# momalekabid/clifford-vae

Hardware: NVIDIA B200
Metric: latent rsample+KL+bind samples/s (higher is better)
Workload: dtype f32

## Files before the change

clifford-vae_b200/clifford_b200/_lib.py:

```python
from __future__ import annotations

import ctypes as C
import os
import threading

import torch

_HERE = os.path.dirname(os.path.abspath(__file__))
LIB_PATH = os.environ.get("CLIFFORD_B200_LIB", os.path.join(_HERE, "libclifford_b200.so"))

_lib = None
_lock = threading.Lock()
_inited_devices: set[int] = set()

_f = C.c_void_p
_ll = C.c_longlong
_ull = C.c_ulonglong
_i = C.c_int
_fl = C.c_float
_db = C.c_double

_SIGNATURES = {
    "cvb_version": ([], _i),
    "cvb_last_error_string": ([], C.c_char_p),
    "cvb_init": ([], _i),
    "cvb_launch_count": ([], _ll),
    "cvb_clifford_ps_rsample": ([_f, _f, _ll, _i, _ll, _f, _f, _ull, _ull, _f, _f, _f, _f, _f, _ll, _i, _f], _i),
    "cvb_clifford_ps_rsample_bind": ([_f, _f, _ll, _f, _f, _ull, _ull, _f, _ll, _f, _f, _f, _f, _f, _ll, _i, _f], _i),
    "cvb_clifford_ps_rsample_log_prob": ([_f, _f, _ll, _f, _f, _ull, _ull, _f, _f, _f, _f, _ll, _i, _f], _i),
    "cvb_clifford_ps_rsample_backward": ([_f, _f, _f, _ll, _i, _ll, _f, _f, _f, _f, _f, _ll, _i, _f], _i),
    "cvb_clifford_ps_log_prob": ([_f, _f, _f, _ll, _i, _ll, _f, _f, _f, _f, _ll, _i, _f], _i),
    "cvb_clifford_spectrum_adjoint": ([_f, _f, _ll, _i, _f], _i),
    "cvb_ps_entropy_kl": ([_f, _ll, _i, _ll, _i, _db, _i, _db, _f, _f, _f, _f], _i),
    "cvb_clifford_vm_rsample": ([_f, _f, _ll, _i, _ll, _ull, _ull, _f, _ll, _i, _f], _i),
    "cvb_clifford_phases_to_vector": ([_f, _fl, _ull, _ull, _f, _ll, _i, _f], _i),
    "cvb_vsa_bind": ([_f, _f, _f, _ll, _ll, _ll, _i, _i, _f], _i),
    "cvb_vsa_depth_chain_cosine": ([_f, _f, _ll, _i, _i, _f], _i),
    "cvb_vsa_invert": ([_f, _f, _ll, _i, _f], _i),
    "cvb_vsa_permute": ([_f, _f, _f, _ll, _i, _i, _f], _i),
    "cvb_vsa_bundle_workspace_bytes": ([_ll, _i], _ll),
    "cvb_vsa_bundle": ([_f, _f, _ll, _i, _fl, _f, _f], _i),
    "cvb_vsa_cosine": ([_f, _f, _f, _ll, _ll, _ll, _i, _f], _i),
    "cvb_vsa_cosine_backward": ([_f, _f, _f, _f, _f, _ll, _ll, _ll, _i, _f], _i),
    "cvb_vsa_normalize": ([_f, _f, _ll, _i, _f], _i),
    "cvb_vsa_normalize_backward": ([_f, _f, _f, _ll, _i, _f], _i),
    "cvb_vsa_hrr_init": ([_f, _ll, _i, _ull, _ull, _f], _i),
    "cvb_vsa_unitary_init": ([_f, _ll, _i, _fl, _ull, _ull, _f], _i),
    "cvb_powerspherical_rsample": ([_f, _f, _ll, _f, _f, _ull, _ull, _f, _f, _ll, _i, _f], _i),
    "cvb_powerspherical_rsample_kl": ([_f, _f, _ll, _f, _f, _ull, _ull, _f, _f, _f, _f, _f, _ll, _i, _f], _i),
    "cvb_powerspherical_rsample_backward": ([_f, _f, _f, _ll, _f, _f, _f, _ull, _ull, _f, _f, _ll, _i, _f], _i),
    "cvb_powerspherical_log_prob": ([_f, _f, _f, _ll, _f, _f, _f, _ll, _i, _f], _i),
    "cvb_ps_log_normalizer": ([_f, _ll, _db, _f, _f, _f], _i),
    "cvb_sphere_uniform_rsample": ([_f, _ull, _ull, _f, _ll, _i, _fl, _f], _i),
    "cvb_vmf_rsample": ([_f, _f, _ll, _f, _f, _i, _f, _ull, _ull, _f, _f, _ll, _i, _f], _i),
    "cvb_vmf_rsample_kl": ([_f, _f, _ll, _f, _f, _i, _f, _ull, _ull, _f, _f, _f, _f, _f, _f, _f, _ll, _i, _f], _i),
    "cvb_vmf_rsample_backward": ([_f, _f, _f, _ll, _f, _f, _ull, _ull, _f, _f, _ll, _i, _f], _i),
    "cvb_vmf_entropy_lognorm": ([_f, _ll, _i, _f, _f, _f, _f, _f], _i),
    "cvb_clifford_ps_rsample_head": ([_f, _f, _ll, _fl, _fl, _f, _f, _ull, _ull, _f, _f, _f, _f, _f, _ll, _i, _f], _i),
    "cvb_clifford_ps_rsample_backward_head": ([_f, _f, _f, _ll, _fl, _fl, _f, _f, _f, _f, _f, _ll, _i, _f], _i),
    "cvb_powerspherical_rsample_kl_head": ([_f, _f, _ll, _fl, _fl, _f, _f, _ull, _ull, _f, _f, _f, _f, _f, _ll, _i, _f], _i),
    "cvb_powerspherical_rsample_backward_head": ([_f, _f, _f, _ll, _fl, _fl, _f, _f, _f, _ull, _ull, _f, _f, _ll, _i, _f], _i),
    "cvb_vmf_rsample_kl_head": ([_f, _f, _ll, _fl, _fl, _f, _f, _i, _f, _ull, _ull, _f, _f, _f, _f, _f, _f, _f, _ll, _i, _f], _i),
    "cvb_vmf_rsample_backward_head": ([_f, _f, _f, _ll, _fl, _fl, _f, _f, _ull, _ull, _f, _f, _ll, _i, _f], _i),
    "cvb_clifford_vm_entropy": ([_f, _ll, _i, _ll, _i, _f, _f, _f], _i),
    "cvb_vmf_log_prob": ([_f, _f, _f, _f, _ll, _f, _f, _ll, _i, _f], _i),
    "cvb_sphere_logprob_backward": ([_f, _f, _f, _ll, _f, _f, _ll, _i, _f], _i),
    "cvb_set_rng_device_counter": ([_f], _i),
    "cvb_set_rng_device_counter_autobump": ([_f], _i),
    "cvb_ps_halfangle_icdf_table": ([_f, _ll, _f, _f, _f], _i),
    "cvb_philox_fill": ([_f, _ll, _ull, _ull, _f], _i),
}

EXPORTED_SYMBOLS = tuple(_SIGNATURES)


class CliffordB200Error(RuntimeError):
    pass


def load():
    global _lib
    if _lib is not None:
        return _lib
    with _lock:
        if _lib is not None:
            return _lib
        if not os.path.exists(LIB_PATH):
            raise CliffordB200Error(
                f"{LIB_PATH} is missing: build it with `python -c 'import __graft_entry__ as g; g.build()'` "
                "(or `make -C clifford-vae_b200/csrc`). There is no CPU / PyTorch fallback for this path.")
        lib = C.CDLL(LIB_PATH)
        for name, (argtypes, restype) in _SIGNATURES.items():
            fn = getattr(lib, name)
            fn.argtypes = argtypes
            fn.restype = restype
        _lib = lib
    return _lib


def ensure_device(device: torch.device) -> None:
    if device.type != "cuda":
        raise CliffordB200Error(
            f"clifford_b200 ops run only on a CUDA (sm_100a) device, got a tensor on '{device}'. "
            "There is deliberately no CPU fallback; move the tensors to the GPU.")
    idx = device.index if device.index is not None else torch.cuda.current_device()
    if idx in _inited_devices:
        return
    lib = load()
    with torch.cuda.device(idx):
        rc = lib.cvb_init()
    if rc != 0:
        raise CliffordB200Error(f"cvb_init failed on cuda:{idx}: {lib.cvb_last_error_string().decode()}")
    _inited_devices.add(idx)


def check(rc: int, what: str) -> None:
    if rc != 0:
        msg = load().cvb_last_error_string().decode()
        if rc == 1:
            raise ValueError(f"{what}: {msg}")
        if rc == 2:
            raise NotImplementedError(f"{what}: {msg}")
# ... 110 lines not shown
```

clifford-vae_b200/csrc/api_core.cu:

```cuda
#include <cstdarg>
#include <cstring>
#include <mutex>
#include <unordered_map>
#include <vector>
#include "launch.cuh"
#include "icdf_table.cuh"
#include "../../include/clifford_b200.h"

namespace cvb {

static thread_local char g_err[512] = "";
std::atomic<long long> g_launch_count{0};
static std::mutex g_mu;
static const cplx* g_tw[64] = {nullptr};
static int g_sms[64] = {0};
static int* g_sched[64] = {nullptr};
static std::atomic<unsigned> g_sched_seq{0};
constexpr int kSchedSlots = 64;
static std::unordered_map<unsigned long long, size_t> g_smem_optin;
static std::unordered_map<unsigned long long, int> g_occ;
static unsigned long long func_key(const void* kernel) {
  int dev = 0;
  cudaGetDevice(&dev);
  return (unsigned long long)reinterpret_cast<uintptr_t>(kernel) * 64ull + (unsigned long long)(dev & 63);
// ... 122 lines not shown

unsigned int* rng_arrive_word() {
  int dev = 0;
  if (cudaGetDevice(&dev) != cudaSuccess || dev < 0 || dev >= 64 || !g_rng_autobump[dev]) return nullptr;
  return g_rng_arrive[dev];
}

int* next_sched_slot() {
  int dev = 0;
  if (cudaGetDevice(&dev) != cudaSuccess || dev < 0 || dev >= 64 || !g_sched[dev]) return nullptr;
  return g_sched[dev] + 2 * (g_sched_seq.fetch_add(1, std::memory_order_relaxed) % kSchedSlots);
}

int sm_count() {
  int dev = 0;
  cudaGetDevice(&dev);
  if (dev >= 0 && dev < 64 && g_sms[dev] > 0) return g_sms[dev];
  int n = 148;
  cudaDeviceGetAttribute(&n, cudaDevAttrMultiProcessorCount, dev);
  if (dev >= 0 && dev < 64) g_sms[dev] = n;
  return n;
}

int cached_ctas_per_sm(const void* kernel, int threads, size_t smem, bool* found) {
  std::lock_guard<std::mutex> lk(g_mu);
  auto it = g_occ.find(occ_key(kernel, threads, smem));
  *found = it != g_occ.end();
  return *found ? it->second : 0;
}
void store_ctas_per_sm(const void* kernel, int threads, size_t smem, int per_sm) {
  std::lock_guard<std::mutex> lk(g_mu);
  g_occ[occ_key(kernel, threads, smem)] = per_sm;
}
int ensure_smem_optin(const void* kernel, size_t smem) {
  if (smem <= 48 * 1024) return kOk;
  std::lock_guard<std::mutex> lk(g_mu);
  size_t& cur = g_smem_optin[func_key(kernel)];
  if (smem > cur) {
    CVB_CUDA(cudaFuncSetAttribute(kernel, cudaFuncAttributeMaxDynamicSharedMemorySize, (int)smem));
    cur = smem;
  }
  return kOk;
}

__global__ void philox_fill_kernel(uint4* out, long long n, PhiloxKey key) {
  for (long long i = (long long)blockIdx.x * blockDim.x + threadIdx.x; i < n; i += (long long)gridDim.x * blockDim.x)
    out[i] = philox4x32_10_rk(make_uint4((uint32_t)i, (uint32_t)(i >> 32), 0u, key.offset), key);
}

}

using namespace cvb;

extern "C" {

int cvb_version(void) { return 100; }
const char* cvb_last_error_string(void) { return g_err; }
long long cvb_launch_count(void) { return g_launch_count.load(); }

int cvb_init(void) {
  int dev = 0;
  CVB_CUDA(cudaGetDevice(&dev));
  CVB_REQUIRE(dev >= 0 && dev < 64, kUnsupported, "device ordinal %d out of range", dev);
  std::lock_guard<std::mutex> lk(g_mu);
  if (g_tw[dev]) return kOk;
  cudaDeviceProp prop;
  CVB_CUDA(cudaGetDeviceProperties(&prop, dev));
  CVB_REQUIRE(prop.major == 10, kUnsupported,
              "clifford_b200 is built for sm_100a only; device %d is sm_%d%d", dev, prop.major, prop.minor);
  std::vector<float2> host(kTwiddleEntries, make_float2(1.f, 0.f));
  for (int L = 4; L <= kTwiddleMaxLog2N; ++L) {
    const int N = 1 << L;
    for (int m = 0; m < N; ++m) {
      const double ang = -2.0 * 3.14159265358979323846264338327950288 * (double)m / (double)(2 * N);
      host[twiddle_offset(L) + m] = make_float2((float)cos(ang), (float)sin(ang));
    }
  }
  cplx* dptr = nullptr;
  CVB_CUDA(cudaMalloc(&dptr, sizeof(cplx) * kTwiddleEntries));
  CVB_CUDA(cudaMemcpy(dptr, host.data(), sizeof(cplx) * kTwiddleEntries, cudaMemcpyHostToDevice));
  int* sched = nullptr;
  CVB_CUDA(cudaMalloc(&sched, sizeof(int) * 2 * kSchedSlots));
  CVB_CUDA(cudaMemset(sched, 0, sizeof(int) * 2 * kSchedSlots));
  if (g_icdf_host.empty()) build_icdf_host(g_icdf_host);
  float2* icdf = nullptr;
  CVB_CUDA(cudaMalloc(&icdf, sizeof(float2) * kIcdfTableEntries));
  {
    std::vector<float2> dev_copy(g_icdf_host);
    for (auto& e : dev_copy) { e.x *= 2.0f; e.y *= 2.0f; }
    CVB_CUDA(cudaMemcpy(icdf, dev_copy.data(), sizeof(float2) * kIcdfTableEntries, cudaMemcpyHostToDevice));
  }
  g_icdf[dev] = icdf;
  g_sched[dev] = sched;
  unsigned int* arrive = nullptr;
  CVB_CUDA(cudaMalloc(&arrive, sizeof(unsigned int)));
  CVB_CUDA(cudaMemset(arrive, 0, sizeof(unsigned int)));
  g_rng_arrive[dev] = arrive;
  g_tw[dev] = dptr;
  g_sms[dev] = prop.multiProcessorCount;
  return kOk;
}

int cvb_set_rng_device_counter(const unsigned long long* counter) {
  int dev = 0;
  CVB_CUDA(cudaGetDevice(&dev));
  CVB_REQUIRE(dev >= 0 && dev < 64, kUnsupported, "device ordinal %d out of range", dev);
  g_rng_ctr[dev] = counter;
  g_rng_autobump[dev] = false;
  return kOk;
}

int cvb_set_rng_device_counter_autobump(unsigned long long* counter) {
  int dev = 0;
  CVB_CUDA(cudaGetDevice(&dev));
  CVB_REQUIRE(dev >= 0 && dev < 64, kUnsupported, "device ordinal %d out of range", dev);
  CVB_REQUIRE(counter == nullptr || g_rng_arrive[dev] != nullptr, kBadArgument, "cvb_set_rng_device_counter_autobump: call cvb_init() first");
  g_rng_ctr[dev] = counter;
  g_rng_autobump[dev] = counter != nullptr;
  return kOk;
}

int cvb_ps_halfangle_icdf_table(float* out, long long capacity_floats, int* n_kappa, int* n_nodes, float* kappa_max) {
  if (n_kappa) *n_kappa = kIcdfKappaNodes;
  if (n_nodes) *n_nodes = kIcdfCells + 1;
  if (kappa_max) *kappa_max = kIcdfKappaMax;
  if (!out) return kOk;
  const long long need = 2LL * kIcdfKappaNodes * (kIcdfCells + 1);
  CVB_REQUIRE(capacity_floats >= need, kBadArgument, "cvb_ps_halfangle_icdf_table: need room for %lld floats", need);
  {
    std::lock_guard<std::mutex> lk(g_mu);
    if (g_icdf_host.empty()) build_icdf_host(g_icdf_host);
  }
  for (int ki = 0; ki < kIcdfKappaNodes; ++ki)
    memcpy(out + 2LL * ki * (kIcdfCells + 1), g_icdf_host.data() + (size_t)ki * kIcdfRowStride, sizeof(float2) * (kIcdfCells + 1));
  return kOk;
}

int cvb_philox_fill(unsigned int* out, long long n_vec4, unsigned long long seed, unsigned long long offset,
                    void* stream) {
  CVB_REQUIRE(out && n_vec4 > 0, kBadArgument, "cvb_philox_fill: bad arguments");
  PhiloxKey key = make_key(seed, 0, 0);
  key.offset = (uint32_t)offset;
  key.dev_counter = nullptr;
  key.arrive = nullptr;
  philox_fill_kernel<<<148, 256, 0, (cudaStream_t)stream>>>(reinterpret_cast<uint4*>(out), n_vec4, key);
  return check_launch("philox_fill_kernel");
}

}
```

clifford-vae_b200/csrc/clifford_kernels.cuh:

```cuda
#pragma once
#include "fft_core.cuh"
#include "tma.cuh"
#include "rng.cuh"
#include "icdf_table.cuh"
#include "special.cuh"
#ifndef CVB_FWD_MINB
#define CVB_FWD_MINB 5
#endif
template <int LOG2N>
constexpr int clifford_bwd_min_blocks() { return LOG2N == 10 ? 4 : 5; }
#ifndef CVB_FWD_BIND_MINB
#define CVB_FWD_BIND_MINB 4
#endif
#ifndef CVB_FWD_KEEP_OWN
#define CVB_FWD_KEEP_OWN 1
#endif
#ifndef CVB_ICDF_LOOP_UNROLL
#define CVB_ICDF_LOOP_UNROLL 4
#endif
#ifndef CVB_FWD_LEAN_MINB
#define CVB_FWD_LEAN_MINB 6
#endif
template <int LOG2N, bool BIND = false, bool LEAN = false>
constexpr int clifford_fwd_min_blocks() {
// ... 465 lines not shown
          if (valid && k != 0) __sincosf(th, &x.y, &x.x);
          xch[pad16(k)] = x;
        }
      }
    } else {
#pragma unroll 4
      for (int e = 0; e < E; ++e) {
        const int k = t + e * T;
        cplx x = make_float2(1.0f, 0.0f);
        if (MODE == kSpectrum) {
          x = make_float2(0.f, 0.f);
          if (valid) {
            clifford_phasor<MODE, ROWK>(p, src, row, prow, k, gm, x);
            if (k == 0) x = make_float2(2.0f * x.x, 0.0f);
          }
        } else if (valid && k != 0) {
          clifford_phasor<MODE, ROWK>(p, src, row, prow, k, gm, x);
          if (MODE == kPsInjected && want_lp) lp_acc += circle_log_half_1pt<false>(src.tprime[k]);
        }
        xch[pad16(k)] = x;
      }
    }
    if (t == 0) xch[pad16(d)] = make_float2(MODE == kSpectrum ? 0.0f : 1.0f, 0.0f);
    if (MODE == kPsInjected && want_lp) lp_reduce();
    group_sync<LOG2N>();
    if (MODE == kPsInjected && want_lp) lp_emit();
    if (ICDF && table_row) {
      if (want_lp) { lp_reduce(); group_sync<LOG2N>(); lp_emit(); }
    } else if (MODE == kPsRng) {
      const int nq = *qcount;
#pragma unroll 1
      for (int i = t; i < nq; i += T) {
        const int k = queue[i];
        float tp_r;
        xch[pad16(k)] = clifford_phasor_retry<ROWK, LEAN>(p, src, row, prow, k, gm, tp_r);
        if (want_lp) lp_acc += circle_log_half_1pt<true>(tp_r);
      }
      if (want_lp) lp_reduce();
      group_sync<LOG2N>();
      if (want_lp) lp_emit();
      if (t == 0) *qcount = 0;
    }
    if (staged && t == 0 && next_row < p.rows) issue(next_row);
    if (ICDF && next_row < p.rows) {
      const float kn = fwd_row_kappa<LEAN || BIND>(p, next_row % p.loc_rows);
      if (icdf_row_ok(kn)) icdf_build_row<false, 1, true>(cells, kn + kEps, icdf, t, T);
    }
    cplx v[E];
    if (BIND) {
#pragma unroll
      for (int e = 0; e < E; ++e) spec[t + e * T] = xch[pad16(t + e * T)];
    }
    if (!BIND || p.z) {
      if constexpr (KEEP_OWN) {
        if (table_row) {
#pragma unroll
          for (int e = 0; e < E; ++e) v[e] = xown[KEEP_OWN ? e : 0];
          c2r_pretangle_load<LOG2N, true>(v, xch, t, tw);
        } else {
          c2r_pretangle_load<LOG2N>(v, xch, t, tw);
        }
      } else {
        c2r_pretangle_load<LOG2N>(v, xch, t, tw);
      }
      fft_run<LOG2N, true>(v, xch, t, tw);
      if (valid) {
        float2* zr = reinterpret_cast<float2*>(p.z + row * (2LL * d));
#pragma unroll
        for (int e = 0; e < E; ++e) stg_stream2(zr + t + e * T, v[e]);
      }
    }
    if (BIND) {
      const float2* br = reinterpret_cast<const float2*>(p.bind_b + (valid ? row % p.bind_b_rows : 0) * (2LL * d));
#pragma unroll
      for (int e = 0; e < E; ++e) v[e] = valid ? ldg_stream2(br + t + e * T) : make_float2(0.f, 0.f);
      fft_run<LOG2N, false>(v, xch, t, tw);
      group_sync<LOG2N>();
#pragma unroll
      for (int e = E / 2; e < E; ++e) xch[pad16(t + e * T)] = v[e];
      group_sync<LOG2N>();
      auto pair = [&](int k, int kp, cplx zb, cplx& vk, cplx& vkp) {
        constexpr float fold = 0.5f / (2.0f * d);
        const cplx zbp = cconj(kp == k ? zb : xch[pad16(kp)]);
        const cplx w = __ldg(&tw[twiddle_offset(LOG2N) + k]);
        const cplx sb = cadd(zb, zbp), db = cmul_mi(cmul(w, csub(zb, zbp)));
        const cplx Bk = cadd(sb, db), Bkp = cconj(csub(sb, db));
        const cplx Pk = cmul(spec[k], Bk), Pkpc = cconj(cmul(spec[kp], Bkp));
        const cplx s = cadd(Pk, Pkpc), q = cmul_i(cmul(cconj(w), csub(Pk, Pkpc)));
        vk = cadd_scaled(s, q, fold);
        vkp = cconj(cscale(csub(s, q), fold));
      };
#pragma unroll
      for (int e = 0; e < E / 2; ++e) {
        const int k = t + e * T, kp = (d - k) & (d - 1);
        cplx vkp;
        pair(k, kp, v[e], v[e], vkp);
        if (kp != k) spec[kp] = vkp;
      }
      if (t == 0) {
        cplx vk, vkp;
        pair(d / 2, d / 2, v[E / 2], vk, vkp);
        spec[d / 2] = vk;
      }
      group_sync<LOG2N>();
#pragma unroll
      for (int e = E / 2; e < E; ++e) v[e] = spec[t + e * T];
// ... 629 lines not shown
```

clifford-vae_b200/csrc/common.cuh:

```cuda
#pragma once
#include <cuda_runtime.h>
#include <cstdint>
#include <cmath>

#ifndef __CUDA_ARCH__
#define CVB_HOST_PASS 1
#endif

namespace cvb {

enum Status : int {
  kOk = 0,
  kBadArgument = 1,
  kUnsupported = 2,
  kCudaError = 3,
};

typedef float2 cplx;

__device__ __forceinline__ cplx cadd(cplx a, cplx b) { return __fadd2_rn(a, b); }
__device__ __forceinline__ cplx csub(cplx a, cplx b) { return __fadd2_rn(a, make_float2(-b.x, -b.y)); }
__device__ __forceinline__ cplx cmul(cplx a, cplx b) {
  return __ffma2_rn(b, make_float2(a.x, a.x), __fmul2_rn(make_float2(b.y, b.x), make_float2(-a.y, a.y)));
}
__device__ __forceinline__ cplx cmulc(cplx a, cplx b) {
  return __ffma2_rn(a, make_float2(b.x, b.x), __fmul2_rn(make_float2(a.y, a.x), make_float2(b.y, -b.y)));
}
__device__ __forceinline__ cplx cconj(cplx a) { return make_float2(a.x, -a.y); }
__device__ __forceinline__ cplx cscale(cplx a, float s) { return __fmul2_rn(a, make_float2(s, s)); }
__device__ __forceinline__ cplx cadd_scaled(cplx a, cplx b, float s) { return __fmul2_rn(__fadd2_rn(a, b), make_float2(s, s)); }
__device__ __forceinline__ cplx caxpy(float s, cplx a, cplx b) { return __ffma2_rn(a, make_float2(s, s), b); }
__device__ __forceinline__ cplx cmul_i(cplx a) { return make_float2(-a.y, a.x); }
__device__ __forceinline__ cplx cmul_mi(cplx a) { return make_float2(a.y, -a.x); }
__device__ __forceinline__ float cabs2(cplx a) { return fmaf(a.x, a.x, a.y * a.y); }

__host__ __device__ __forceinline__ constexpr int pad16(int i) { return i + (i >> 4); }

constexpr int kTwiddleMaxLog2N = 13;
constexpr int kTwiddleEntries = 1 << (kTwiddleMaxLog2N + 1);
__host__ __device__ __forceinline__ constexpr int twiddle_offset(int log2n) { return 1 << log2n; }

__device__ __forceinline__ float2 ldg_stream2(const float2* p) {
  float2 r;
  asm volatile("ld.global.nc.L1::no_allocate.v2.f32 {%0, %1}, [%2];" : "=f"(r.x), "=f"(r.y) : "l"(p));
  return r;
}
__device__ __forceinline__ float ldg_stream1(const float* p) {
  float r;
  asm volatile("ld.global.nc.L1::no_allocate.f32 %0, [%1];" : "=f"(r) : "l"(p));
  return r;
}
__device__ __forceinline__ void stg_stream2(float2* p, float2 v) {
  asm volatile("st.global.L1::no_allocate.v2.f32 [%0], {%1, %2};" ::"l"(p), "f"(v.x), "f"(v.y) : "memory");
}
__device__ __forceinline__ void stg_stream1(float* p, float v) {
  asm volatile("st.global.L1::no_allocate.f32 [%0], %1;" ::"l"(p), "f"(v) : "memory");
}

__device__ __forceinline__ void pdl_wait_and_release() {
  asm volatile("griddepcontrol.wait;" ::: "memory");
  asm volatile("griddepcontrol.launch_dependents;" ::: "memory");
}

__device__ __forceinline__ float fast_sqrt(float x) {
  float r;
  asm("sqrt.approx.ftz.f32 %0, %1;" : "=f"(r) : "f"(x));
  return r;
}

struct KappaHead {
  int on;
  float floor, kmax;
};
__device__ __forceinline__ float head_kappa(const KappaHead& h, float raw) {
  if (!h.on) return raw;
  const float sp = raw > 20.0f ? raw : log1pf(expf(raw));
  return fminf(sp + h.floor, h.kmax);
}
__device__ __forceinline__ float head_dkappa(const KappaHead& h, float raw) {
  if (!h.on) return 1.0f;
  const float e = expf(raw);
  const float sp = raw > 20.0f ? raw : log1pf(e);
  if (!(sp + h.floor <= h.kmax)) return 0.0f;
  return raw > 20.0f ? 1.0f : e / (e + 1.0f);
}

__device__ __forceinline__ float warp_sum(float v) {
#pragma unroll
  for (int o = 16; o > 0; o >>= 1) v += __shfl_xor_sync(0xffffffffu, v, o);
  return v;
}
__device__ __forceinline__ double warp_sum(double v) {
#pragma unroll
// ... 6 lines not shown
```

clifford-vae_b200/csrc/fft_core.cuh:

```cuda
#pragma once
#include "common.cuh"

namespace cvb {

constexpr int default_loge(int log2n) { return (log2n >= 8) ? 4 : (log2n >= 6 ? 3 : 2); }

template <int LOG2N_, int LOGE_, int MINTHREADS_ = 128>
struct FftPlanT {
  static_assert(LOG2N_ >= 4 && LOG2N_ <= 13, "fast path covers N = 16 .. 8192 complex points");
  static constexpr int LOG2N = LOG2N_;
  static constexpr int N = 1 << LOG2N;
  static constexpr int LOGE = LOGE_;
  static constexpr int E = 1 << LOGE;
  static constexpr int T = N / E;
  static constexpr int LOGT = LOG2N - LOGE;
  static constexpr int XCH = pad16(N) + 2;
  static constexpr int THREADS = (T >= MINTHREADS_) ? T : MINTHREADS_;
  static constexpr int GROUPS = THREADS / T;
};
template <int LOG2N>
using FftPlan = FftPlanT<LOG2N, default_loge(LOG2N)>;
template <int LOG2N>
using WideFftPlan = FftPlanT<LOG2N, (LOG2N >= 13) ? 5 : default_loge(LOG2N)>;

template <class Pl>
__device__ __forceinline__ void group_sync_p() {
  if constexpr (Pl::T <= 32) {
    __syncwarp();
  } else if constexpr (Pl::T < Pl::THREADS) {
    asm volatile("bar.sync %0, %1;" ::"r"(1 + (int)(threadIdx.x / Pl::T)), "n"(Pl::T) : "memory");
  } else {
    __syncthreads();
  }
}
template <int LOG2N>
__device__ __forceinline__ void group_sync() { group_sync_p<FftPlan<LOG2N>>(); }

template <bool INV>
__device__ __forceinline__ void dft2(cplx& a, cplx& b) {
  cplx t = a;
  a = cadd(t, b);
  b = csub(t, b);
}

template <bool INV>
__device__ __forceinline__ void dft4(cplx& a0, cplx& a1, cplx& a2, cplx& a3) {
  cplx s0 = cadd(a0, a2), d0 = csub(a0, a2);
  cplx s1 = cadd(a1, a3), d1 = csub(a1, a3);
  cplx r = INV ? cmul_i(d1) : cmul_mi(d1);
  a0 = cadd(s0, s1);
  a2 = csub(s0, s1);
  a1 = cadd(d0, r);
  a3 = csub(d0, r);
}

template <bool INV>
__device__ __forceinline__ cplx rot(cplx z, float c, float s) {
  return INV ? __ffma2_rn(z, make_float2(c, c), __fmul2_rn(make_float2(z.y, z.x), make_float2(-s, s)))
             : __ffma2_rn(z, make_float2(c, c), __fmul2_rn(make_float2(z.y, z.x), make_float2(s, -s)));
}

template <int R, bool INV>
struct Dft;

template <bool INV>
struct Dft<2, INV> {
  static __device__ __forceinline__ void run(cplx (&u)[2]) { dft2<INV>(u[0], u[1]); }
};
template <bool INV>
struct Dft<4, INV> {
  static __device__ __forceinline__ void run(cplx (&u)[4]) { dft4<INV>(u[0], u[1], u[2], u[3]); }
};
template <bool INV>
struct Dft<8, INV> {
  static __device__ __forceinline__ void run(cplx (&u)[8]) {
    constexpr float h = 0.70710678118654752440f;
    dft4<INV>(u[0], u[2], u[4], u[6]);
    dft4<INV>(u[1], u[3], u[5], u[7]);
    cplx o0 = u[1];
    cplx o1 = rot<INV>(u[3], h, h);
    cplx o2 = INV ? cmul_i(u[5]) : cmul_mi(u[5]);
    cplx o3 = rot<INV>(u[7], -h, h);
    cplx e0 = u[0], e1 = u[2], e2 = u[4], e3 = u[6];
    u[0] = cadd(e0, o0); u[4] = csub(e0, o0);
    u[1] = cadd(e1, o1); u[5] = csub(e1, o1);
    u[2] = cadd(e2, o2); u[6] = csub(e2, o2);
    u[3] = cadd(e3, o3); u[7] = csub(e3, o3);
  }
};
template <bool INV>
struct Dft<16, INV> {
  static __device__ __forceinline__ void run(cplx (&u)[16]) {
    constexpr float c1 = 0.92387953251128675613f, s1 = 0.38268343236508977173f;
    constexpr float h = 0.70710678118654752440f;
#pragma unroll
    for (int n1 = 0; n1 < 4; ++n1) dft4<INV>(u[n1], u[n1 + 4], u[n1 + 8], u[n1 + 12]);
    u[5] = rot<INV>(u[5], c1, s1);
    u[6] = rot<INV>(u[6], h, h);
    u[7] = rot<INV>(u[7], s1, c1);
    u[9] = rot<INV>(u[9], h, h);
    u[10] = INV ? cmul_i(u[10]) : cmul_mi(u[10]);
    u[11] = rot<INV>(u[11], -h, h);
    u[13] = rot<INV>(u[13], s1, c1);
    u[14] = rot<INV>(u[14], -h, h);
    u[15] = rot<INV>(u[15], -c1, -s1);
#pragma unroll
    for (int k2 = 0; k2 < 4; ++k2) dft4<INV>(u[4 * k2], u[4 * k2 + 1], u[4 * k2 + 2], u[4 * k2 + 3]);
    cplx t;
#define CVB_SWAP(a, b) t = u[a]; u[a] = u[b]; u[b] = t;
    CVB_SWAP(1, 4) CVB_SWAP(2, 8) CVB_SWAP(3, 12) CVB_SWAP(6, 9) CVB_SWAP(7, 13) CVB_SWAP(11, 14)
#undef CVB_SWAP
  }
};

template <bool INV>
struct Dft<32, INV> {
  static __device__ __forceinline__ void run(cplx (&u)[32]) {
    constexpr float c[16] = {1.0f, 0.98078528040323044913f, 0.92387953251128675613f, 0.83146961230254523708f,
                             0.70710678118654752440f, 0.55557023301960222474f, 0.38268343236508977173f, 0.19509032201612826785f,
                             0.0f, -0.19509032201612826785f, -0.38268343236508977173f, -0.55557023301960222474f,
                             -0.70710678118654752440f, -0.83146961230254523708f, -0.92387953251128675613f, -0.98078528040323044913f};
    constexpr float s[16] = {0.0f, 0.19509032201612826785f, 0.38268343236508977173f, 0.55557023301960222474f,
                             0.70710678118654752440f, 0.83146961230254523708f, 0.92387953251128675613f, 0.98078528040323044913f,
                             1.0f, 0.98078528040323044913f, 0.92387953251128675613f, 0.83146961230254523708f,
                             0.70710678118654752440f, 0.55557023301960222474f, 0.38268343236508977173f, 0.19509032201612826785f};
    cplx ev[16], od[16];
#pragma unroll
    for (int i = 0; i < 16; ++i) { ev[i] = u[2 * i]; od[i] = u[2 * i + 1]; }
    Dft<16, INV>::run(ev);
    Dft<16, INV>::run(od);
#pragma unroll
    for (int k = 0; k < 16; ++k) {
      cplx o;
      if (k == 0) o = od[0];
      else if (k == 8) o = INV ? cmul_i(od[8]) : cmul_mi(od[8]);
      else o = rot<INV>(od[k], c[k], s[k]);
      u[k] = cadd(ev[k], o);
      u[k + 16] = csub(ev[k], o);
    }
  }
};


template <bool INV>
struct Dft<64, INV> {
  static __device__ __forceinline__ void run(cplx (&u)[64]) {
    constexpr float C[17] = {1.0f, 0.99518472667219688624f, 0.98078528040323044913f, 0.95694033573220886494f,
                             0.92387953251128675613f, 0.88192126434835502971f, 0.83146961230254523708f, 0.77301045336273696081f,
                             0.70710678118654752440f, 0.63439328416364549822f, 0.55557023301960222474f, 0.47139673682599764856f,
                             0.38268343236508977173f, 0.29028467725446236764f, 0.19509032201612826785f, 0.09801714032956060199f, 0.0f};
#pragma unroll
    for (int n1 = 0; n1 < 8; ++n1) {
      cplx w[8];
#pragma unroll
      for (int j = 0; j < 8; ++j) w[j] = u[n1 + 8 * j];
      Dft<8, INV>::run(w);
#pragma unroll
      for (int j = 0; j < 8; ++j) u[n1 + 8 * j] = w[j];
    }
#pragma unroll
    for (int n1 = 1; n1 < 8; ++n1) {
#pragma unroll
      for (int k2 = 1; k2 < 8; ++k2) {
        const int m = n1 * k2;
        const int q = m >> 4, r = m & 15;
        const float c0 = C[r], s0 = C[16 - r];
        const float c = (q == 0) ? c0 : (q == 1) ? -s0 : (q == 2) ? -c0 : s0;
        const float sn = (q == 0) ? s0 : (q == 1) ? c0 : (q == 2) ? -s0 : -c0;
        cplx& z = u[n1 + 8 * k2];
        if (r == 0) {
          z = (q == 1) ? (INV ? cmul_i(z) : cmul_mi(z)) : (q == 2) ? make_float2(-z.x, -z.y) : (INV ? cmul_mi(z) : cmul_i(z));
        } else {
          z = rot<INV>(z, c, sn);
        }
      }
    }
#pragma unroll
    for (int k2 = 0; k2 < 8; ++k2) {
      cplx w[8];
#pragma unroll
      for (int j = 0; j < 8; ++j) w[j] = u[8 * k2 + j];
      Dft<8, INV>::run(w);
#pragma unroll
      for (int j = 0; j < 8; ++j) u[8 * k2 + j] = w[j];
    }
#pragma unroll
    for (int a = 0; a < 8; ++a) {
#pragma unroll
      for (int b = a + 1; b < 8; ++b) {
        const cplx tmp = u[a + 8 * b];
        u[a + 8 * b] = u[b + 8 * a];
        u[b + 8 * a] = tmp;
      }
    }
  }
};

template <int R>
__device__ __forceinline__ void apply_twiddle_powers(cplx (&u)[R], cplx w1) {
  if constexpr (R > 16) {
    cplx pw = w1, cur = w1;
#pragma unroll
    for (int i = 1; i < R; ++i) {
      if (i > 1) {
        if ((i & (i - 1)) == 0) { pw = cmul(pw, pw); cur = pw; }
        else cur = cmul(cur, w1);
      }
      u[i] = cmul(u[i], cur);
    }
    return;
  }
  cplx w[R];
  w[1] = w1;
#pragma unroll
  for (int i = 2; i < R; ++i) {
    if (i & 1) {
      w[i] = cmul(w[i - 1], w1);
    } else {
      w[i] = cmul(w[i >> 1], w[i >> 1]);
    }
  }
#pragma unroll
  for (int i = 1; i < R; ++i) u[i] = cmul(u[i], w[i]);
}

template <class Pl>
__device__ __forceinline__ void load_own_points(cplx (&v)[Pl::E], const cplx* xch, int t) {
  if constexpr (Pl::T % 16 == 0) {
    constexpr int S = Pl::T + Pl::T / 16;
    const cplx* xr = xch + pad16(t);
#pragma unroll
    for (int e = 0; e < Pl::E; ++e) v[e] = xr[e * S];
  } else {
#pragma unroll
    for (int e = 0; e < Pl::E; ++e) v[e] = xch[pad16(t + e * Pl::T)];
  }
}

template <class Pl, int P, bool INV, bool BASEPTR = false>
__device__ __forceinline__ void fft_pass_p(cplx (&v)[Pl::E], cplx* xch, const int t, const cplx* __restrict__ tw) {
  constexpr int LOG2N = Pl::LOG2N;
  constexpr int LOGNS = P * Pl::LOGE;
  constexpr int LOGR = (LOG2N - LOGNS) < Pl::LOGE ? (LOG2N - LOGNS) : Pl::LOGE;
  constexpr int R = 1 << LOGR, Q = Pl::E / R, NS = 1 << LOGNS;
  constexpr bool LAST = (LOGNS + LOGR == LOG2N);
  if (!LAST) group_sync_p<Pl>();
#pragma unroll
  for (int q = 0; q < Q; ++q) {
    cplx u[R];
#pragma unroll
    for (int r = 0; r < R; ++r) u[r] = v[q + r * Q];
    const int j = t + q * Pl::T;
    const int k = j & (NS - 1);
    if (P > 0) {
      cplx w1 = __ldg(&tw[twiddle_offset(LOG2N) + (k << (LOG2N + 1 - LOGNS - LOGR))]);
      if (INV) w1.y = -w1.y;
      apply_twiddle_powers<R>(u, w1);
    }
    Dft<R, INV>::run(u);
    if (LAST) {
#pragma unroll
      for (int r = 0; r < R; ++r) v[q + r * Q] = u[r];
    } else {
      const int j0 = ((j - k) << LOGR) + k;
#pragma unroll
      for (int r = 0; r < R; ++r) xch[pad16(j0 + r * NS)] = u[r];
    }
  }
  if constexpr (!LAST) {
    group_sync_p<Pl>();
    if constexpr (BASEPTR) {
      load_own_points<Pl>(v, xch, t);
    } else {
#pragma unroll
      for (int e = 0; e < Pl::E; ++e) v[e] = xch[pad16(t + e * Pl::T)];
    }
    fft_pass_p<Pl, P + 1, INV, BASEPTR>(v, xch, t, tw);
  }
}

template <class Pl, bool INV>
__device__ __forceinline__ void fft_run_p(cplx (&v)[Pl::E], cplx* xch, int t, const cplx* __restrict__ tw) {
  fft_pass_p<Pl, 0, INV>(v, xch, t, tw);
}
template <int LOG2N, bool INV>
__device__ __forceinline__ void fft_run(cplx (&v)[FftPlan<LOG2N>::E], cplx* xch, int t,
                                        const cplx* __restrict__ tw) {
  fft_pass_p<FftPlan<LOG2N>, 0, INV, true>(v, xch, t, tw);
}

template <int LOG2N>
__device__ __forceinline__ float r2c_untangle(cplx (&v)[FftPlan<LOG2N>::E], cplx* xch, int t,
                                              const cplx* __restrict__ tw) {
  using Pl = FftPlan<LOG2N>;
  constexpr int N = Pl::N;
  if constexpr (Pl::T % 16 == 0) {
    constexpr int S = Pl::T + Pl::T / 16;
    cplx* xk = xch + pad16(t);
    const cplx* xm = xch + pad16(N - t);
    const cplx* twp = tw + twiddle_offset(LOG2N) + t;
    group_sync<LOG2N>();
#pragma unroll
    for (int e = 0; e < Pl::E; ++e) xk[e * S] = v[e];
    group_sync<LOG2N>();
    const float nyq0 = v[0].x - v[0].y;
#pragma unroll
    for (int e = 0; e < Pl::E; ++e) {
      const cplx z = v[e];
      const cplx* pp = (e == 0) ? ((t == 0) ? xch : xm) : xm - e * S;
      const cplx zp = cconj(*pp);
      const cplx w = __ldg(twp + e * Pl::T);
      const cplx s = cadd(z, zp), d = csub(z, zp);
      const cplx wd = cmul_mi(cmul(w, d));
      v[e] = cadd_scaled(s, wd, 0.5f);
    }
    return nyq0;
  }
  group_sync<LOG2N>();
#pragma unroll
  for (int e = 0; e < Pl::E; ++e) xch[pad16(t + e * Pl::T)] = v[e];
  group_sync<LOG2N>();
  const float nyq = v[0].x - v[0].y;
#pragma unroll
  for (int e = 0; e < Pl::E; ++e) {
    const int k = t + e * Pl::T;
    const cplx z = v[e];
    const cplx zp = cconj(xch[pad16((N - k) & (N - 1))]);
    const cplx w = __ldg(&tw[twiddle_offset(LOG2N) + k]);
    const cplx s = cadd(z, zp), d = csub(z, zp);
    const cplx wd = cmul_mi(cmul(w, d));
    v[e] = cadd_scaled(s, wd, 0.5f);
  }
  return nyq;
}

template <int LOG2N>
__device__ __forceinline__ void c2r_pretangle(cplx (&v)[FftPlan<LOG2N>::E], float x_nyq, cplx* xch, int t,
                                              const cplx* __restrict__ tw) {
  using Pl = FftPlan<LOG2N>;
  constexpr int N = Pl::N;
  constexpr float scale = 1.0f / (2.0f * N);
  group_sync<LOG2N>();
#pragma unroll
  for (int e = 0; e < Pl::E; ++e) xch[pad16(t + e * Pl::T)] = v[e];
  if (t == 0) xch[pad16(N)] = make_float2(x_nyq, 0.0f);
  group_sync<LOG2N>();
#pragma unroll
  for (int e = 0; e < Pl::E; ++e) {
    const int k = t + e * Pl::T;
    const cplx x = v[e];
    const cplx xp = cconj(xch[pad16(N - k)]);
    const cplx w = cconj(__ldg(&tw[twiddle_offset(LOG2N) + k]));
    const cplx s = cadd(x, xp), d = csub(x, xp);
    const cplx wd = cmul_i(cmul(w, d));
    v[e] = cadd_scaled(s, wd, scale);
  }
}

template <int LOG2N, bool OWN = false>
__device__ __forceinline__ void c2r_pretangle_load(cplx (&v)[FftPlan<LOG2N>::E], const cplx* xch, int t,
                                                   const cplx* __restrict__ tw) {
  using Pl = FftPlan<LOG2N>;
  constexpr int N = Pl::N;
  constexpr float scale = 1.0f / (2.0f * N);
  if constexpr (Pl::T % 16 == 0) {
    constexpr int S = Pl::T + Pl::T / 16;
    const cplx* xk = xch + pad16(t);
    const cplx* xm = xch + pad16(N - t);
    const cplx* twp = tw + twiddle_offset(LOG2N) + t;
#pragma unroll
    for (int e = 0; e < Pl::E; ++e) {
      const cplx x = OWN ? v[e] : xk[e * S];
      const cplx xp = cconj(xm[-e * S]);
      const cplx w = cconj(__ldg(twp + e * Pl::T));
      const cplx s = cadd(x, xp), d = csub(x, xp);
      const cplx wd = cmul_i(cmul(w, d));
      v[e] = cadd_scaled(s, wd, scale);
    }
    return;
  }
#pragma unroll
  for (int e = 0; e < Pl::E; ++e) {
    const int k = t + e * Pl::T;
    const cplx x = OWN ? v[e] : xch[pad16(k)];
    const cplx xp = cconj(xch[pad16(N - k)]);
    const cplx w = cconj(__ldg(&tw[twiddle_offset(LOG2N) + k]));
    const cplx s = cadd(x, xp), d = csub(x, xp);
    const cplx wd = cmul_i(cmul(w, d));
    v[e] = cadd_scaled(s, wd, scale);
  }
}

template <int LOG2N>
__device__ __forceinline__ float group_sum(float val, float* scratch, int t) {
  constexpr int T = FftPlan<LOG2N>::T;
  constexpr int W = T < 32 ? T : 32;
#pragma unroll
  for (int o = W / 2; o > 0; o >>= 1) val += __shfl_xor_sync(0xffffffffu, val, o);
  if constexpr (T > 32) {
    group_sync<LOG2N>();
    if ((t & 31) == 0) scratch[t >> 5] = val;
    group_sync<LOG2N>();
    float s = 0.f;
#pragma unroll
    for (int i = 0; i < T / 32; ++i) s += scratch[i];
    val = s;
  }
  return val;
}

}
```

include/clifford_b200.h:

```cpp
#ifndef CLIFFORD_B200_H_
#define CLIFFORD_B200_H_

#if defined(__GNUC__)
#define CVB_API __attribute__((visibility("default")))
#else
#define CVB_API
#endif

#ifdef __cplusplus
extern "C" {
#endif

enum cvb_status { CVB_OK = 0, CVB_BAD_ARGUMENT = 1, CVB_UNSUPPORTED = 2, CVB_CUDA_ERROR = 3 };

enum cvb_bind_mode {
  CVB_BIND_MUL = 0,
  CVB_BIND_MUL_CONJ = 1,
  CVB_BIND_DIV = 2,
  CVB_BIND_DIV_CONJ = 3,
  CVB_BIND_NEG_MUL_CONJ = 4
};

CVB_API int cvb_version(void);
CVB_API const char* cvb_last_error_string(void);
// ... 81 lines not shown
                            unsigned long long offset, float* z, float* save, long long rows, int D, void* stream);
CVB_API int cvb_vmf_rsample_kl(const float* loc, const float* kappa, long long loc_rows, const double* e_rounds,
                               const double* u_rounds, int n_rounds, const float* gnoise, unsigned long long seed,
                               unsigned long long offset, float* z, float* save, float* entropy, float* kl,
                               float* dentropy, float* log_norm, float* dlog_norm, long long rows, int D, void* stream);
CVB_API int cvb_vmf_rsample_backward(const float* grad_z, const float* loc, const float* kappa, long long loc_rows,
                                     const float* gnoise, const float* save, unsigned long long seed,
                                     unsigned long long offset, float* dloc, float* dkappa, long long rows, int D,
                                     void* stream);
CVB_API int cvb_vmf_entropy_lognorm(const float* kappa, long long rows, int D, float* entropy, float* log_norm,
                                    float* dentropy, float* dlog_norm, void* stream);

CVB_API int cvb_clifford_vm_entropy(const float* kappa, long long kappa_row_stride, int kappa_el_stride, long long rows,
                                    int d, float* entropy, float* dentropy, void* stream);
CVB_API int cvb_vmf_log_prob(const float* value, const float* loc, const float* kappa, const float* log_norm,
                             long long loc_rows, float* log_prob, float* dot, long long rows, int D, void* stream);
CVB_API int cvb_sphere_logprob_backward(const float* w, const float* value, const float* loc, long long loc_rows,
                                        float* dvalue, float* dloc, long long rows, int D, void* stream);

CVB_API int cvb_clifford_ps_rsample_head(const float* loc, const float* raw_scale, long long loc_rows, float floor, float kmax,
                                         const float* tprime, const float* gnoise, unsigned long long seed,
                                         unsigned long long offset, float* z, float* tp_signed, float* entropy, float* kl,
                                         float* dentropy_draw, long long rows, int d, void* stream);
CVB_API int cvb_clifford_ps_rsample_backward_head(const float* grad_z, const float* loc, const float* raw_scale,
                                                  long long loc_rows, float floor, float kmax, const float* tprime,
                                                  const float* gnoise, const float* tp_signed, float* dloc,
                                                  float* draw_scale, long long rows, int d, void* stream);
CVB_API int cvb_powerspherical_rsample_kl_head(const float* loc, const float* raw_scale, long long loc_rows, float floor,
                                               float kmax, const float* tprime, const float* gnoise,
                                               unsigned long long seed, unsigned long long offset, float* z, float* save,
                                               float* entropy, float* kl, float* dentropy_draw, long long rows, int D,
                                               void* stream);
CVB_API int cvb_powerspherical_rsample_backward_head(const float* grad_z, const float* loc, const float* raw_scale,
                                                     long long loc_rows, float floor, float kmax, const float* tprime,
                                                     const float* gnoise, const float* save, unsigned long long seed,
                                                     unsigned long long offset, float* dloc, float* draw_scale,
                                                     long long rows, int D, void* stream);
CVB_API int cvb_vmf_rsample_kl_head(const float* loc, const float* raw_scale, long long loc_rows, float floor, float kmax,
                                    const double* e_rounds, const double* u_rounds, int n_rounds, const float* gnoise,
                                    unsigned long long seed, unsigned long long offset, float* z, float* save,
                                    float* entropy, float* kl, float* dentropy_draw, float* log_norm,
                                    float* dlog_norm_draw, long long rows, int D, void* stream);
CVB_API int cvb_vmf_rsample_backward_head(const float* grad_z, const float* loc, const float* raw_scale, long long loc_rows,
                                          float floor, float kmax, const float* gnoise, const float* save,
                                          unsigned long long seed, unsigned long long offset, float* dloc,
                                          float* draw_scale, long long rows, int D, void* stream);

CVB_API int cvb_set_rng_device_counter(const unsigned long long* counter);
CVB_API int cvb_set_rng_device_counter_autobump(unsigned long long* counter);

CVB_API int cvb_ps_halfangle_icdf_table(float* out, long long capacity_floats, int* n_kappa, int* n_nodes,
                                        float* kappa_max);

CVB_API int cvb_philox_fill(unsigned int* out, long long n_vec4, unsigned long long seed, unsigned long long offset,
                    void* stream);

#ifdef __cplusplus
}
#endif
#endif
```

Baseline: 34.16 million.

## Precompute FFT stage twiddle powers in table and restructure radix-8/16 butterflies with FMAs

```diff
diff --git a/clifford-vae_b200/clifford_b200/_lib.py b/clifford-vae_b200/clifford_b200/_lib.py
--- a/clifford-vae_b200/clifford_b200/_lib.py
+++ b/clifford-vae_b200/clifford_b200/_lib.py
@@ -68,6 +68,7 @@
     "cvb_set_rng_device_counter": ([_f], _i),
     "cvb_set_rng_device_counter_autobump": ([_f], _i),
     "cvb_ps_halfangle_icdf_table": ([_f, _ll, _f, _f, _f], _i),
+    "cvb_fft_twiddle_table": ([_f, _ll, _f], _i),
     "cvb_philox_fill": ([_f, _ll, _ull, _ull, _f], _i),
 }
 
diff --git a/clifford-vae_b200/csrc/api_core.cu b/clifford-vae_b200/csrc/api_core.cu
--- a/clifford-vae_b200/csrc/api_core.cu
+++ b/clifford-vae_b200/csrc/api_core.cu
@@ -198,6 +198,32 @@
 
 using namespace cvb;
 
+static float2 unit_root(long long m, long long M) {
+  const long long q = (4 * m) / M, r = m - q * (M / 4);
+  const double a = 2.0 * 3.14159265358979323846264338327950288 * (double)r / (double)M;
+  const double c = cos(a), s = -sin(a);
+  const double x = (q == 0) ? c : (q == 1) ? s : (q == 2) ? -c : -s;
+  const double y = (q == 0) ? s : (q == 1) ? -c : (q == 2) ? -s : c;
+  return make_float2((float)x, (float)y);
+}
+
+static void build_twiddle_host(std::vector<float2>& host) {
+  host.assign(kTwiddleTableEntries, make_float2(1.f, 0.f));
+  for (int L = 4; L <= kTwiddleMaxLog2N; ++L) {
+    const int N = 1 << L;
+    for (int m = 0; m < N; ++m) {
+      const double ang = -2.0 * 3.14159265358979323846264338327950288 * (double)m / (double)(2 * N);
+      host[twiddle_offset(L) + m] = make_float2((float)cos(ang), (float)sin(ang));
+    }
+  }
+  for (int logr = 1; logr <= kPowerMaxLog2R; ++logr)
+    for (int logns = 1; logns + logr <= kTwiddleMaxLog2N; ++logns) {
+      const int NS = 1 << logns, R = 1 << logr;
+      for (int j = 0; j < logr; ++j)
+        for (int k = 0; k < NS; ++k) host[power_offset(logns, logr) + j * NS + k] = unit_root((long long)k << j, (long long)NS * R);
+    }
+}
+
 extern "C" {
 
 int cvb_version(void) { return 100; }
@@ -214,17 +240,11 @@
   CVB_CUDA(cudaGetDeviceProperties(&prop, dev));
   CVB_REQUIRE(prop.major == 10, kUnsupported,
               "clifford_b200 is built for sm_100a only; device %d is sm_%d%d", dev, prop.major, prop.minor);
-  std::vector<float2> host(kTwiddleEntries, make_float2(1.f, 0.f));
-  for (int L = 4; L <= kTwiddleMaxLog2N; ++L) {
-    const int N = 1 << L;
-    for (int m = 0; m < N; ++m) {
-      const double ang = -2.0 * 3.14159265358979323846264338327950288 * (double)m / (double)(2 * N);
-      host[twiddle_offset(L) + m] = make_float2((float)cos(ang), (float)sin(ang));
-    }
-  }
+  std::vector<float2> host;
+  build_twiddle_host(host);
   cplx* dptr = nullptr;
-  CVB_CUDA(cudaMalloc(&dptr, sizeof(cplx) * kTwiddleEntries));
-  CVB_CUDA(cudaMemcpy(dptr, host.data(), sizeof(cplx) * kTwiddleEntries, cudaMemcpyHostToDevice));
+  CVB_CUDA(cudaMalloc(&dptr, sizeof(cplx) * kTwiddleTableEntries));
+  CVB_CUDA(cudaMemcpy(dptr, host.data(), sizeof(cplx) * kTwiddleTableEntries, cudaMemcpyHostToDevice));
   int* sched = nullptr;
   CVB_CUDA(cudaMalloc(&sched, sizeof(int) * 2 * kSchedSlots));
   CVB_CUDA(cudaMemset(sched, 0, sizeof(int) * 2 * kSchedSlots));
@@ -282,6 +302,17 @@
   return kOk;
 }
 
+int cvb_fft_twiddle_table(float* out, long long capacity_floats, long long* n_entries) {
+  if (n_entries) *n_entries = kTwiddleTableEntries;
+  if (!out) return kOk;
+  CVB_REQUIRE(capacity_floats >= 2LL * kTwiddleTableEntries, kBadArgument,
+              "cvb_fft_twiddle_table: need room for %lld floats", 2LL * kTwiddleTableEntries);
+  std::vector<float2> host;
+  build_twiddle_host(host);
+  memcpy(out, host.data(), sizeof(float2) * kTwiddleTableEntries);
+  return kOk;
+}
+
 int cvb_philox_fill(unsigned int* out, long long n_vec4, unsigned long long seed, unsigned long long offset,
                     void* stream) {
   CVB_REQUIRE(out && n_vec4 > 0, kBadArgument, "cvb_philox_fill: bad arguments");
diff --git a/clifford-vae_b200/csrc/clifford_kernels.cuh b/clifford-vae_b200/csrc/clifford_kernels.cuh
--- a/clifford-vae_b200/csrc/clifford_kernels.cuh
+++ b/clifford-vae_b200/csrc/clifford_kernels.cuh
@@ -541,6 +541,9 @@
       for (int e = 0; e < E; ++e) spec[t + e * T] = xch[pad16(t + e * T)];
     }
     if (!BIND || p.z) {
+#ifdef CVB_PAIR_PRETANGLE
+      if (BIND) group_sync<LOG2N>();
+#endif
       if constexpr (KEEP_OWN) {
         if (table_row) {
 #pragma unroll
diff --git a/clifford-vae_b200/csrc/common.cuh b/clifford-vae_b200/csrc/common.cuh
--- a/clifford-vae_b200/csrc/common.cuh
+++ b/clifford-vae_b200/csrc/common.cuh
@@ -39,6 +39,14 @@
 constexpr int kTwiddleMaxLog2N = 13;
 constexpr int kTwiddleEntries = 1 << (kTwiddleMaxLog2N + 1);
 __host__ __device__ __forceinline__ constexpr int twiddle_offset(int log2n) { return 1 << log2n; }
+
+constexpr int kPowerMaxLog2R = 4;
+__host__ __device__ __forceinline__ constexpr int power_offset(int logns, int logr) {
+  int off = kTwiddleEntries;
+  for (int b = 1; b < logr; ++b) off += b * ((1 << (kTwiddleMaxLog2N + 1 - b)) - 2);
+  return off + logr * ((1 << logns) - 2);
+}
+constexpr int kTwiddleTableEntries = power_offset(kTwiddleMaxLog2N + 1 - kPowerMaxLog2R, kPowerMaxLog2R);
 
 __device__ __forceinline__ float2 ldg_stream2(const float2* p) {
   float2 r;
diff --git a/clifford-vae_b200/csrc/fft_core.cuh b/clifford-vae_b200/csrc/fft_core.cuh
--- a/clifford-vae_b200/csrc/fft_core.cuh
+++ b/clifford-vae_b200/csrc/fft_core.cuh
@@ -72,40 +72,67 @@
   static __device__ __forceinline__ void run(cplx (&u)[4]) { dft4<INV>(u[0], u[1], u[2], u[3]); }
 };
 template <bool INV>
+__device__ __forceinline__ cplx jrot(cplx z) { return INV ? cmul_i(z) : cmul_mi(z); }
+__device__ __forceinline__ void fma_pm(cplx a, cplx z, float s, cplx& plus, cplx& minus) {
+  plus = __ffma2_rn(z, make_float2(s, s), a);
+  minus = __ffma2_rn(z, make_float2(-s, -s), a);
+}
+
+template <bool INV>
 struct Dft<8, INV> {
   static __device__ __forceinline__ void run(cplx (&u)[8]) {
     constexpr float h = 0.70710678118654752440f;
     dft4<INV>(u[0], u[2], u[4], u[6]);
     dft4<INV>(u[1], u[3], u[5], u[7]);
-    cplx o0 = u[1];
-    cplx o1 = rot<INV>(u[3], h, h);
-    cplx o2 = INV ? cmul_i(u[5]) : cmul_mi(u[5]);
-    cplx o3 = rot<INV>(u[7], -h, h);
-    cplx e0 = u[0], e1 = u[2], e2 = u[4], e3 = u[6];
+    const cplx o1 = cadd(u[3], jrot<INV>(u[3]));
+    const cplx o2 = jrot<INV>(u[5]);
+    const cplx o3 = csub(jrot<INV>(u[7]), u[7]);
+    const cplx o0 = u[1];
+    const cplx e0 = u[0], e1 = u[2], e2 = u[4], e3 = u[6];
     u[0] = cadd(e0, o0); u[4] = csub(e0, o0);
-    u[1] = cadd(e1, o1); u[5] = csub(e1, o1);
+    fma_pm(e1, o1, h, u[1], u[5]);
     u[2] = cadd(e2, o2); u[6] = csub(e2, o2);
-    u[3] = cadd(e3, o3); u[7] = csub(e3, o3);
+    fma_pm(e3, o3, h, u[3], u[7]);
   }
 };
 template <bool INV>
 struct Dft<16, INV> {
   static __device__ __forceinline__ void run(cplx (&u)[16]) {
-    constexpr float c1 = 0.92387953251128675613f, s1 = 0.38268343236508977173f;
+    constexpr float c1 = 0.92387953251128675613f;
+    constexpr float tn = 0.41421356237309504880f;
     constexpr float h = 0.70710678118654752440f;
 #pragma unroll
     for (int n1 = 0; n1 < 4; ++n1) dft4<INV>(u[n1], u[n1 + 4], u[n1 + 8], u[n1 + 12]);
-    u[5] = rot<INV>(u[5], c1, s1);
-    u[6] = rot<INV>(u[6], h, h);
-    u[7] = rot<INV>(u[7], s1, c1);
-    u[9] = rot<INV>(u[9], h, h);
-    u[10] = INV ? cmul_i(u[10]) : cmul_mi(u[10]);
-    u[11] = rot<INV>(u[11], -h, h);
-    u[13] = rot<INV>(u[13], s1, c1);
-    u[14] = rot<INV>(u[14], -h, h);
-    u[15] = rot<INV>(u[15], -c1, -s1);
-#pragma unroll
-    for (int k2 = 0; k2 < 4; ++k2) dft4<INV>(u[4 * k2], u[4 * k2 + 1], u[4 * k2 + 2], u[4 * k2 + 3]);
+    dft4<INV>(u[0], u[1], u[2], u[3]);
+    {
+      const cplx a2 = cadd(u[6], jrot<INV>(u[6]));
+      cplx s0, d0;
+      fma_pm(u[4], a2, h, s0, d0);
+      const cplx b1 = __ffma2_rn(jrot<INV>(u[5]), make_float2(tn, tn), u[5]);
+      const cplx b3 = __ffma2_rn(u[7], make_float2(tn, tn), jrot<INV>(u[7]));
+      const cplx s1 = cadd(b1, b3), d1 = csub(b1, b3);
+      fma_pm(s0, s1, c1, u[4], u[6]);
+      fma_pm(d0, jrot<INV>(d1), c1, u[5], u[7]);
+    }
+    {
+      const cplx a2 = jrot<INV>(u[10]);
+      const cplx s0 = cadd(u[8], a2), d0 = csub(u[8], a2);
+      const cplx b1 = cadd(u[9], jrot<INV>(u[9]));
+      const cplx b3 = csub(jrot<INV>(u[11]), u[11]);
+      const cplx s1 = cadd(b1, b3), d1 = csub(b1, b3);
+      fma_pm(s0, s1, h, u[8], u[10]);
+      fma_pm(d0, jrot<INV>(d1), h, u[9], u[11]);
+    }
+    {
+      const cplx a2 = csub(jrot<INV>(u[14]), u[14]);
+      cplx s0, d0;
+      fma_pm(u[12], a2, h, s0, d0);
+      const cplx b1 = __ffma2_rn(u[13], make_float2(tn, tn), jrot<INV>(u[13]));
+      const cplx b3 = __ffma2_rn(jrot<INV>(u[15]), make_float2(tn, tn), u[15]);
+      const cplx s1 = csub(b1, b3), d1 = cadd(b1, b3);
+      fma_pm(s0, s1, c1, u[12], u[14]);
+      fma_pm(d0, jrot<INV>(d1), c1, u[13], u[15]);
+    }
     cplx t;
 #define CVB_SWAP(a, b) t = u[a]; u[a] = u[b]; u[b] = t;
     CVB_SWAP(1, 4) CVB_SWAP(2, 8) CVB_SWAP(3, 12) CVB_SWAP(6, 9) CVB_SWAP(7, 13) CVB_SWAP(11, 14)
@@ -198,30 +225,30 @@
 
 template <int R>
 __device__ __forceinline__ void apply_twiddle_powers(cplx (&u)[R], cplx w1) {
-  if constexpr (R > 16) {
-    cplx pw = w1, cur = w1;
-#pragma unroll
-    for (int i = 1; i < R; ++i) {
-      if (i > 1) {
-        if ((i & (i - 1)) == 0) { pw = cmul(pw, pw); cur = pw; }
-        else cur = cmul(cur, w1);
-      }
-      u[i] = cmul(u[i], cur);
-    }
-    return;
-  }
+  cplx pw = w1, cur = w1;
+#pragma unroll
+  for (int i = 1; i < R; ++i) {
+    if (i > 1) {
+      if ((i & (i - 1)) == 0) { pw = cmul(pw, pw); cur = pw; }
+      else cur = cmul(cur, w1);
+    }
+    u[i] = cmul(u[i], cur);
+  }
+}
+
+template <int R, int NS, bool INV>
+__device__ __forceinline__ void apply_table_powers(cplx (&u)[R], const cplx* __restrict__ pw) {
   cplx w[R];
-  w[1] = w1;
-#pragma unroll
-  for (int i = 2; i < R; ++i) {
-    if (i & 1) {
-      w[i] = cmul(w[i - 1], w1);
-    } else {
-      w[i] = cmul(w[i >> 1], w[i >> 1]);
-    }
-  }
-#pragma unroll
-  for (int i = 1; i < R; ++i) u[i] = cmul(u[i], w[i]);
+#pragma unroll
+  for (int r = 1, j = 0; r < R; r *= 2, ++j) w[r] = __ldg(pw + j * NS);
+#pragma unroll
+  for (int r = 3; r < R; ++r) {
+    int hi = 1;
+    while (2 * hi <= r) hi *= 2;
+    if (r != hi) w[r] = cmul(w[hi], w[r - hi]);
+  }
+#pragma unroll
+  for (int r = 1; r < R; ++r) u[r] = INV ? cmulc(u[r], w[r]) : cmul(u[r], w[r]);
 }
 
 template <class Pl>
@@ -252,10 +279,15 @@
     for (int r = 0; r < R; ++r) u[r] = v[q + r * Q];
     const int j = t + q * Pl::T;
     const int k = j & (NS - 1);
-    if (P > 0) {
+#ifndef CVB_CHAIN
+#define CVB_CHAIN 0
+#endif
+    if constexpr (P > 0 && (R > 16 || CVB_CHAIN == 2 || (CVB_CHAIN == 1 && BASEPTR))) {
       cplx w1 = __ldg(&tw[twiddle_offset(LOG2N) + (k << (LOG2N + 1 - LOGNS - LOGR))]);
       if (INV) w1.y = -w1.y;
       apply_twiddle_powers<R>(u, w1);
+    } else if constexpr (P > 0) {
+      apply_table_powers<R, NS, INV>(u, tw + power_offset(LOGNS, LOGR) + k);
     }
     Dft<R, INV>::run(u);
     if (LAST) {
@@ -357,6 +389,36 @@
   }
 }
 
+#ifdef CVB_PAIR_PRETANGLE
+template <int LOG2N, bool OWN = false>
+__device__ __forceinline__ void c2r_pretangle_load(cplx (&v)[FftPlan<LOG2N>::E], cplx* xch, int t,
+                                                   const cplx* __restrict__ tw) {
+  using Pl = FftPlan<LOG2N>;
+  constexpr int N = Pl::N, T = Pl::T, E = Pl::E, S = T + T / 16;
+  constexpr float scale = 1.0f / (2.0f * N);
+  auto own = [&](int e) -> cplx* { return (T % 16 == 0) ? xch + pad16(t) + e * S : xch + pad16(t + e * T); };
+  auto par = [&](int e) -> cplx* { return (T % 16 == 0) ? xch + pad16(N - t) - e * S : xch + pad16(N - t - e * T); };
+  const cplx* twp = tw + twiddle_offset(LOG2N) + t;
+#pragma unroll
+  for (int e = 0; e < E / 2; ++e) {
+    const cplx x = OWN ? v[e] : *own(e);
+    const cplx xp = cconj(*par(e));
+    const cplx w = cconj(__ldg(twp + e * T));
+    const cplx s = cadd(x, xp), q = cmul_i(cmul(w, csub(x, xp)));
+    v[e] = cadd_scaled(s, q, scale);
+    if (e > 0 || t > 0) *par(e) = cconj(cscale(csub(s, q), scale));
+  }
+  if (t == 0) {
+    const cplx x = OWN ? v[E / 2] : *own(E / 2);
+    const cplx xp = cconj(x);
+    const cplx w = cconj(__ldg(twp + (E / 2) * T));
+    *own(E / 2) = cadd_scaled(cadd(x, xp), cmul_i(cmul(w, csub(x, xp))), scale);
+  }
+  group_sync<LOG2N>();
+#pragma unroll
+  for (int e = E / 2; e < E; ++e) v[e] = *own(e);
+}
+#else
 template <int LOG2N, bool OWN = false>
 __device__ __forceinline__ void c2r_pretangle_load(cplx (&v)[FftPlan<LOG2N>::E], const cplx* xch, int t,
                                                    const cplx* __restrict__ tw) {
@@ -390,6 +452,7 @@
     v[e] = cadd_scaled(s, wd, scale);
   }
 }
+#endif
 
 template <int LOG2N>
 __device__ __forceinline__ float group_sum(float val, float* scratch, int t) {
diff --git a/include/clifford_b200.h b/include/clifford_b200.h
--- a/include/clifford_b200.h
+++ b/include/clifford_b200.h
@@ -157,6 +157,8 @@
 CVB_API int cvb_ps_halfangle_icdf_table(float* out, long long capacity_floats, int* n_kappa, int* n_nodes,
                                         float* kappa_max);
 
+CVB_API int cvb_fft_twiddle_table(float* out, long long capacity_floats, long long* n_entries);
+
 CVB_API int cvb_philox_fill(unsigned int* out, long long n_vec4, unsigned long long seed, unsigned long long offset,
                     void* stream);
 
```

Result: faster. 34.78 million, median of 6 (+1.8%).
